# YanhaoWu/UMGen

Measured on AMD Instinct MI355X. Metric: scene_tokens_per_sec, higher is better.
Workload: dtype bf16; 1 GPU; UMGen_large --infer_task video, 5-frame rollout, 1 scene(s)/GPU, T=20 history frames, top-k 5/5/16 sampling, rule_constrain; scenes_per_gpu=1, history_frames=20, input_history_frames=20

## Files before the change

umgen_amd/csrc/debug_gemm_attn.hip:

```cpp
#include "debug_util.h"

namespace {
GemmArgs linear_args(const void* dW, const void* dA, int R, int N, int K, void* dO) {
    GemmArgs g{};
    g.P = dW; g.Q = dA; g.Mi = N; g.Nj = R; g.K = K; g.ldp = K; g.ldq = K; g.batch = 1; g.out = dO; g.ldo = N;
    return g;
}
GemmArgs vt_args(const void* dA, const void* dW, int F, int S, int S_pad, int N, int K, void* dO) {
    GemmArgs g{};
    g.P = dA; g.Q = dW; g.Mi = S; g.Nj = N; g.K = K; g.ldp = K; g.ldq = K; g.strideP = (long)S * K; g.strideQ = 0; g.batch = F;
    g.mode = GEMM_VT; g.out = dO; g.ldo = S_pad; g.H = N / kHeadDim;
    return g;
}
inline int pad64(int S) { return ((S + 63) / 64) * 64; }
void lcg_operands(Scratch& s, size_t na, size_t nw, DevPtr& dA, DevPtr& dW) {
    std::vector<bf16_t> h;
    unsigned x = 12345u;
    fill_lcg(h, na, x, 1.0f);
    dA = s.in(h.data(), na * 2);
    fill_lcg(h, nw, x, 0.05f);
    dW = s.in(h.data(), nw * 2);
}
}

extern "C" {

int umgen_dbg_linear(int flags, const void* act, const void* W, const float* bias, int R, int N, int K, int gelu, int resid, void* out) {
    const int bf16 = flags & 3;
    const size_t es = bf16 ? 2 : 4, osz = (size_t)R * N * (resid ? 4 : es);
    Scratch s;
    const void *dA = s.in(act, (size_t)R * K * es), *dW = s.in(W, (size_t)N * K * es);
    const float* dB = s.in(bias, (size_t)N * 4);
    void* dO = resid ? s.in(out, osz) : s.raw((size_t)R * N * 4);
    if (s.rc) return s.rc;
    GemmArgs g = linear_args(dW, dA, R, N, K, dO);
    g.mode = resid ? GEMM_RESID : GEMM_STORE; g.bias = dB; g.gelu = gelu;
    g.tile256 = (flags & 16) ? 1 : ((flags & 32) ? -1 : 0);
    if (bf16) by_prec16(bf16, [&](auto t) { launch_gemm_mfma<decltype(t)>(nullptr, g); });
    else launch_gemm_valu<float, float>(nullptr, g);
    if (int rc = finish()) return rc;
    return down(out, dO, osz);
}

int umgen_dbg_linear_vt(int flags, const void* act, const void* W, const float* bias, int F, int S, int N, int K, void* out) {
    const int prec = flags & 3;
    if (prec != 1 && prec != 2) return UMGEN_E_UNSUPPORTED;
    const int S_pad = pad64(S);
    const size_t R = (size_t)F * S, osz = (size_t)F * N * S_pad * 2;
    Scratch s;
    const void *dA = s.in(act, R * K * 2), *dW = s.in(W, (size_t)N * K * 2);
    const float* dB = s.in(bias, (size_t)N * 4);
    void* dO = s.raw(osz);
    if (s.rc) return s.rc;
    (void)hipMemset(dO, 0, osz);
    GemmArgs g = vt_args(dA, dW, F, S, S_pad, N, K, dO);
    g.bias = dB;
    g.tile256 = (flags & 16) ? 1 : ((flags & 32) ? -1 : 0);
    by_prec16(prec, [&](auto t) { launch_gemm_mfma<decltype(t)>(nullptr, g); });
    if (int rc = finish()) return rc;
    return down(out, dO, osz);
}

int umgen_dbg_attn_spatial(int flags, const void* qk, const void* v, int F, int S, int H, void* y) {
    const int bf16 = flags & 3;
    if ((flags & 64) && (flags & 32)) return UMGEN_E_UNSUPPORTED;
    const int E = H * kHeadDim, S_pad = pad64(S);
    const size_t es = bf16 ? 2 : 4, R = (size_t)F * S;
    std::vector<unsigned char> vt((size_t)F * E * S_pad * es, 0);
    const unsigned char* vs = (const unsigned char*)v;
    for (int f = 0; f < F; ++f)
        for (int sr = 0; sr < S; ++sr)
            for (int c = 0; c < E; ++c)
                memcpy(&vt[(((size_t)f * E + c) * S_pad + sr) * es], &vs[(((size_t)f * S + sr) * E + c) * es], es);
    Scratch s;
    const void *dQK = s.in(qk, R * 2 * E * es), *dVT = s.in(vt.data(), vt.size());
    void* dY = s.out(R * E * es);
    if (s.rc) return s.rc;
    if (int rc = fill_nan(dY, R * E, bf16)) return rc;
    by_prec(bf16, [&](auto t) {
        typedef decltype(t) T;
        const T *q = (const T*)dQK, *vtp = (const T*)dVT;
        if constexpr (std::is_same<T, float>::value) {
            if (flags & 64) launch_attn_causal_f32(nullptr, q, vtp, (T*)dY, F, S, S_pad, H);
            else if (flags & 32) launch_attn_spatial_valu<float>(nullptr, q, vtp, (T*)dY, F, S, S_pad, H);
            else launch_attn_spatial_f32_mfma(nullptr, q, vtp, (T*)dY, F, S, S_pad, H);
        } else if (flags & 64) {
            launch_attn_causal_mfma<T>(nullptr, q, vtp, (T*)dY, F, S, S_pad, H);
        } else {
            launch_attn_spatial_mfma<T>(nullptr, q, vtp, (T*)dY, F, S, S_pad, H);
        }
    });
    if (int rc = s.finish()) return rc;
    return down(y, dY, R * E * es);
}

int umgen_dbg_attn_temporal(int bf16, const void* qkv, int B, int T, int S, int H, int split, void* y) {
    const int E = H * kHeadDim;
    const size_t es = bf16 ? 2 : 4, row = (size_t)3 * E * es, orow = (size_t)E * es;
    auto pass = [&](int t0, int Tn, TemporalRange tr) -> int {
        const size_t Rn = (size_t)B * Tn * S;
        std::vector<unsigned char> hq(Rn * row), hy(Rn * orow);
        for (int b = 0; b < B; ++b)
            memcpy(&hq[(size_t)b * Tn * S * row], (const unsigned char*)qkv + ((size_t)b * T + t0) * S * row, (size_t)Tn * S * row);
        Scratch s;
        const void* dQ = s.in(hq.data(), hq.size());
        void* dY = s.raw(hy.size());
        if (s.rc) return s.rc;
        by_prec(bf16, [&](auto t) { typedef decltype(t) TT; launch_attn_temporal<TT>(nullptr, (const TT*)dQ, (TT*)dY, B, Tn, S, H, tr); });
        if (int rc = finish()) return rc;
        if (down(hy.data(), dY, hy.size())) return UMGEN_E_HIP;
        for (int b = 0; b < B; ++b)
            memcpy((unsigned char*)y + ((size_t)b * T + t0) * S * orow, &hy[(size_t)b * Tn * S * orow], (size_t)Tn * S * orow);
        return UMGEN_OK;
    };
    if (split <= 0 || split >= T) return pass(0, T, TemporalRange{0, nullptr, 0, 0});
    const int Tcap = T + 1;
    Scratch s;
    void* dC = s.raw((size_t)B * Tcap * S * 2 * E * es);
    if (s.rc) return s.rc;
    if (int rc = pass(0, split, TemporalRange{0, dC, Tcap, 1})) return rc;
    return pass(split, T - split, TemporalRange{split, dC, Tcap, 0});
}

int umgen_dbg_attn_decode(int bf16, const float* q, const void* kv, int NQ, int L, int H, float* y) {
    const int E = H * kHeadDim;
    const size_t es = bf16 ? 2 : 4;
    std::vector<float> eye((size_t)E * E, 0.f);
    for (int i = 0; i < E; ++i) eye[(size_t)i * E + i] = 1.f;
    Scratch s;
    const float* dQ = s.in(q, (size_t)NQ * E * 4);
    const void *dKV = s.in(kv, (size_t)L * 2 * E * es), *dW = s.in(eye.data(), eye.size() * 4);
    float *dP = s.raw((size_t)NQ * H * kAttnRec * 4), *dX = s.raw((size_t)NQ * E * 4);
    if (s.rc) return s.rc;
    (void)hipMemset(dX, 0, (size_t)NQ * E * 4);
    by_prec(bf16, [&](auto t) {
        typedef decltype(t) T;
        launch_attn_partial<T>(nullptr, dQ, (const T*)dKV, 0, kHeadDim, 2L * E, E, NQ, NQ, H, nullptr, L, attn_nsplit(L), dP);
    });
    GemvResidArgs a{};
    a.part = dP; a.H = H; a.ns = attn_nsplit(L); a.W = dW; a.N = E; a.K = E; a.M = NQ; a.x = dX; a.ldx = E;
    launch_gemv_resid<float>(nullptr, a);
    if (int rc = finish()) return rc;
    return down(y, dX, (size_t)NQ * E * 4);
}

int umgen_dbg_gemm_bench(int R, int N, int K, int mode, int iters, float* ms) {
    Scratch s;
    DevPtr dA, dW;
    lcg_operands(s, (size_t)R * K, (size_t)N * K, dA, dW);
    void* dO = s.raw((size_t)R * N * 4);
    if (s.rc) return s.rc;
    (void)hipMemset(dO, 0, (size_t)R * N * 4);
    GemmArgs g = linear_args(dW, dA, R, N, K, dO);
    g.mode = mode & 15; g.gelu = (mode >> 4) & 1;
    g.tile256 = (mode & 64) ? -1 : ((mode & 32) ? 1 : 0);
    return time_launches(nullptr, 1, iters, 1, ms, [&](int) { launch_gemm_mfma<bf16_t>(nullptr, g); });
}

int umgen_dbg_gemm_vt_bench(int F, int S, int N, int K, int flag, int iters, float* ms) {
    const int S_pad = pad64(S);
    const size_t osz = (size_t)F * N * S_pad * 2;
    Scratch s;
    DevPtr dA, dW;
    lcg_operands(s, (size_t)F * S * K, (size_t)N * K, dA, dW);
    void* dO = s.raw(osz);
    if (s.rc) return s.rc;
    (void)hipMemset(dO, 0, osz);
    GemmArgs g = vt_args(dA, dW, F, S, S_pad, N, K, dO);
    g.tile256 = (flag & 64) ? -1 : ((flag & 32) ? 1 : 0);
    return time_launches(nullptr, 1, iters, 1, ms, [&](int) { launch_gemm_mfma<bf16_t>(nullptr, g); });
}

int umgen_dbg_gemm_stamps(unsigned long long* out16) { return gemm256_read_stamps(out16); }

int umgen_dbg_gemv(int bf16, const float* x, const float* ln_w, const void* W, const float* bias, int M, int N, int K, int gelu, float* out) {
    const size_t es = bf16 ? 2 : 4, osz = (size_t)M * N * 4;
    Scratch s;
    GemvArgs a{};
    a.x = s.in(x, (size_t)M * K * 4); a.ldx = K; a.ln_w = s.in(ln_w, (size_t)K * 4); a.W = s.in(W, (size_t)N * K * es); a.bias = s.in(bias, (size_t)N * 4);
    a.N = N; a.K = K; a.M = M; a.out_mode = gelu ? GEMV_OUT_GELU : GEMV_OUT_F32; a.out = s.raw(osz); a.ldo = N; a.E = K;
    if (s.rc) return s.rc;
    for (int rpb = 0; rpb <= (M > 1 ? 1 : 0); ++rpb) {
        std::vector<float> got((size_t)M * N);
        if (rpb) (void)hipMemset(a.out, 0, osz);
        a.rows_per_block = rpb;
        by_prec(bf16, [&](auto t) { launch_gemv<decltype(t)>(nullptr, a); });
        if (int rc = finish()) return rc;
        if (int rc = down(rpb ? got.data() : out, a.out, osz)) return rc;
        if (rpb && memcmp(got.data(), out, osz) != 0) return UMGEN_E_STATE;
    }
    return UMGEN_OK;
}

int umgen_dbg_sample_topk(const float* logits, int n, int V, int k, float temp, const float* u, int32_t* tokens, int32_t* overflow) {
    if (V > 8192 || V < 1 || n < 1) return UMGEN_E_INVALID;
    Scratch s;
    const float *dL = s.in(logits, (size_t)n * V * 4), *dU = s.in(u, (size_t)n * 4);
    int *dT = s.raw((size_t)n * 4), *dO = s.raw(4);
    if (s.rc) return s.rc;
    (void)hipMemset(dO, 0, 4);
    launch_sample_rows(nullptr, dL, V, k, temp, dU, dT, dO, n);
    if (int rc = finish()) return rc;
    if (int rc = down(tokens, dT, (size_t)n * 4)) return rc;
    return down(overflow, dO, 4);
}

int umgen_dbg_batched_layer_bench(int prec, int M, int L, int iters, float* us) {
    const int E = 768, H = 16, Lmax = 2304;
    if (prec != 1 && prec != 2) return UMGEN_E_INVALID;
    if (M < 1 || M > kRowsMaxM || L < 1 || L >= Lmax) return UMGEN_E_INVALID;
    const size_t wsz = (size_t)12 * E * E * 2, csz = (size_t)M * 2 * H * Lmax * kHeadDim * 2, xsz = (size_t)64 * E * 4;
    std::vector<unsigned short> hw(wsz / 2);
    for (size_t i = 0; i < hw.size(); ++i) hw[i] = (unsigned short)(0x3c00 + (i * 2654435761u >> 24)) & (prec == 1 ? 0x3cff : 0x2fff);
    std::vector<float> hx((size_t)64 * E, 0.25f), hl(E, 1.f), hb(4 * E, 0.f);
    for (size_t i = 0; i < hx.size(); ++i) hx[i] = 0.25f + 1e-3f * (float)(i % 97);
    Scratch s;
    const char* Wq = s.in(hw.data(), wsz);
    void* dC = s.raw(csz);
    float *dx = s.in(hx.data(), xsz), *dxr = s.in(hx.data(), xsz), *dq = s.raw(xsz), *da = s.raw(xsz), *dh = s.raw(4 * xsz);
    const float *dln = s.in(hl.data(), (size_t)E * 4), *db = s.in(hb.data(), (size_t)4 * E * 4);
    const int* dlen = s.in(&L, 4);
    if (s.rc) return s.rc;
    if (hipMemset(da, 0, xsz) != hipSuccess || hipMemset(dh, 0, 4 * xsz) != hipSuccess || hipMemset(dC, 0, csz) != hipSuccess) return UMGEN_E_HIP;
    Stream stream;
    if (!stream.s) return UMGEN_E_HIP;
    hipStream_t st = stream.s;
    const long cstride = (long)2 * H * Lmax * kHeadDim;
    auto run = [&](int which) {
        by_prec16(prec, [&](auto tag) {
            typedef decltype(tag) TT;
            RowsArgs r{};
            r.M = M; r.E = E;
            switch (which) {
                case 0: r.x = dx; r.ln_w = dln; r.W = Wq; r.bias = db; r.N = 3 * E; r.K = E; r.mode = ROWS_QKV; r.out = dq; r.ldo = E;
                        r.cache = dC; r.scene_stride = cstride; r.d_len = dlen; r.Lmax = Lmax; launch_rows_mfma<TT>(st, r); break;
                case 1: launch_attn_decode_batched<TT>(st, dq, (const TT*)dC, cstride, M, H, Lmax, dlen, da); break;
                case 2: r.x = da; r.W = Wq + (size_t)3 * E * E * 2; r.bias = db; r.N = E; r.K = E; r.mode = ROWS_RESID; r.out = dxr; r.ldo = E; r.out_frag = dx; launch_rows_mfma<TT>(st, r); break;
                case 3: r.x = dx; r.ln_w = dln; r.W = Wq + (size_t)4 * E * E * 2; r.N = 4 * E; r.K = E; r.mode = ROWS_GELU; r.out_frag = dh; launch_rows_mfma<TT>(st, r); break;
                default: r.x = dh; r.W = Wq + (size_t)8 * E * E * 2; r.N = E; r.K = 4 * E; r.mode = ROWS_RESID; r.out = dxr; r.ldo = E; r.out_frag = dx; launch_rows_mfma<TT>(st, r); break;
            }
        });
    };
    if (int rc = time_launches(st, 3, iters, 6, us, [&](int which) { if (which < 5) run(which); else for (int k = 0; k < 5; ++k) run(k); })) return rc;
    for (int i = 0; i < 6; ++i) us[i] *= 1000.f;
    return UMGEN_OK;
}

}
```

umgen_amd/csrc/gemm.hip:

```cpp
#include <cstdlib>

#include "bg_queue.h"
#include "kernels.h"

namespace umgen {

template <int MODE, typename TO>
__device__ inline void epilogue4(const GemmArgs& a, int z, int i0, int j, const float (&v)[4]) {
    if (j >= a.Nj || i0 >= a.Mi) return;
    if (MODE == GEMM_VT) {
        const float b = a.bias ? a.bias[j] : 0.f;
        TO* dst = reinterpret_cast<TO*>(a.out) + (((long)z * a.H + j / kHeadDim) * kHeadDim + j % kHeadDim) * a.ldo + i0;
        if (i0 + 3 < a.Mi) {
            float o[4] = {v[0] + b, v[1] + b, v[2] + b, v[3] + b};
            store4(dst, o);
        } else {
            for (int r = 0; r < 4 && i0 + r < a.Mi; ++r) dst[r] = Cvt<TO>::from_f(v[r] + b);
        }
        return;
    }
    float o[4];
#pragma unroll
    for (int r = 0; r < 4; ++r) {
        float t = v[r] + (a.bias ? a.bias[i0 + r] : 0.f);
// ... 43 lines not shown
        pp[it] = P + (long)gi * a.ldp + schunk * 8;
        qq[it] = Q + (long)gj * a.ldq + schunk * 8;
    }
    uint4 rp[4], rq[4];
    auto gload = [&](int k0) {
        const bool ok = (k0 + schunk * 8) < a.K;
#pragma unroll
        for (int it = 0; it < 4; ++it) {
            rp[it] = ok ? *reinterpret_cast<const uint4*>(pp[it] + k0) : make_uint4(0, 0, 0, 0);
            rq[it] = ok ? *reinterpret_cast<const uint4*>(qq[it] + k0) : make_uint4(0, 0, 0, 0);
        }
    };
    auto lstore = [&](int buf) {
        unsigned char* ldsP = lds[buf];
        unsigned char* ldsQ = lds[buf] + BM * BK * 2;
#pragma unroll
        for (int it = 0; it < 4; ++it) {
            int r = srow + 32 * it;
            *reinterpret_cast<uint4*>(ldsP + swz(r, schunk)) = rp[it];
            *reinterpret_cast<uint4*>(ldsQ + swz(r, schunk)) = rq[it];
        }
    };
    f32x4_t acc[4][4];
#pragma unroll
    for (int m = 0; m < 4; ++m)
#pragma unroll
        for (int n = 0; n < 4; ++n) acc[m][n] = f32x4_t{0.f, 0.f, 0.f, 0.f};

    const int frow = lane & 15, g = lane >> 4;
    const int nkt = (a.K + BK - 1) / BK;
    gload(0);
    lstore(0);
    if (nkt > 1) gload(BK);
    __syncthreads();
    for (int kt = 0; kt < nkt; ++kt) {
        const unsigned char* ldsP = lds[kt & 1];
        const unsigned char* ldsQ = lds[kt & 1] + BM * BK * 2;
#pragma unroll
        for (int kk = 0; kk < 2; ++kk) {
            vec8 af[4], bfr[4];
            const int c = kk * 4 + g;
#pragma unroll
            for (int m = 0; m < 4; ++m) af[m] = *reinterpret_cast<const vec8*>(ldsP + swz(wi * 64 + m * 16 + frow, c));
#pragma unroll
            for (int n = 0; n < 4; ++n) bfr[n] = *reinterpret_cast<const vec8*>(ldsQ + swz(wj * 64 + n * 16 + frow, c));
#pragma unroll
            for (int m = 0; m < 4; ++m)
#pragma unroll
                for (int n = 0; n < 4; ++n) acc[m][n] = Mma16<TT>::mfma(af[m], bfr[n], acc[m][n]);
        }
        if (kt + 1 < nkt) {
            lstore((kt + 1) & 1);
            if (kt + 2 < nkt) gload((kt + 2) * BK);
        }
        __syncthreads();
    }
#pragma unroll
    for (int m = 0; m < 4; ++m)
#pragma unroll
        for (int n = 0; n < 4; ++n) {
            const int i0 = i_base + wi * 64 + m * 16 + 4 * g;
            const int j = j_base + wj * 64 + n * 16 + frow;
            float v[4] = {acc[m][n][0], acc[m][n][1], acc[m][n][2], acc[m][n][3]};
            epilogue4<MODE, TT>(a, z, i0, j, v);
        }
}

template <typename TT>
__device__ __forceinline__ void store_tile_rows_bf16(const GemmArgs& a, int z, int ti, int tj, const f32x4_t (&acc)[4][2], unsigned char* stg,
                                                     int tid, int wi, int wj, int frow, int g) {
    asm volatile("" ::: "memory");
    __builtin_amdgcn_s_barrier();
#pragma unroll
    for (int m = 0; m < 4; ++m) {
        const int i0 = ti * BM + wi * 64 + m * 16 + 4 * g;
        float bb[4];
#pragma unroll
        for (int r = 0; r < 4; ++r) bb[r] = a.bias ? a.bias[i0 + r] : 0.f;
#pragma unroll
        for (int n = 0; n < 2; ++n) {
            float o[4];
#pragma unroll
            for (int r = 0; r < 4; ++r) {
                const float t = acc[m][n][r] + bb[r];
                o[r] = a.gelu ? gelu_fast(t) : t;
            }
            const int tl = wj * 32 + n * 16 + frow;
            const int pg = (wi * 16 + m * 4 + g) ^ frow;
            store4(reinterpret_cast<TT*>(stg + tl * 256 + pg * 8), o);
        }
    }
    asm volatile("s_waitcnt lgkmcnt(0)" ::: "memory");
    __builtin_amdgcn_s_barrier();
    TT* out = reinterpret_cast<TT*>(a.out) + (long)z * a.strideO + (long)ti * BM;
#pragma unroll
    for (int it = 0; it < 4; ++it) {
        const int idx = tid + 512 * it;
        const int tl = idx >> 4, q = idx & 15;
        const int pos = ((2 * q) ^ (tl & 15)) & ~1;
        uint4 v = *reinterpret_cast<const uint4*>(stg + tl * 256 + pos * 8);
        if (tl & 1) v = make_uint4(v.z, v.w, v.x, v.y);
        const int token = tj * BN + tl;
        if (token < a.Nj) {
            typedef unsigned int u32x4 __attribute__((ext_vector_type(4)));
            __builtin_nontemporal_store(u32x4{v.x, v.y, v.z, v.w}, reinterpret_cast<u32x4*>(out + (long)token * a.ldo + 8 * q));
        }
    }
    asm volatile("s_waitcnt lgkmcnt(0)" ::: "memory");
}

__device__ __forceinline__ void rmw_tile_rows_f32(const GemmArgs& a, int z, int ti, int tj, const f32x4_t (&acc)[4][2], unsigned char* stg,
                                                  int tid, int wi, int wj, int frow, int g) {
    float* xbase = reinterpret_cast<float*>(a.out) + (long)z * a.strideO + (long)ti * BM;
#pragma unroll
    for (int hf = 0; hf < 2; ++hf) {
        asm volatile("s_waitcnt lgkmcnt(0)" ::: "memory");
        __builtin_amdgcn_s_barrier();
        if ((wj >> 1) == hf) {
#pragma unroll
            for (int m = 0; m < 4; ++m) {
                const int i0 = ti * BM + wi * 64 + m * 16 + 4 * g;
                float bb[4];
#pragma unroll
                for (int r = 0; r < 4; ++r) bb[r] = a.bias ? a.bias[i0 + r] : 0.f;
#pragma unroll
                for (int n = 0; n < 2; ++n) {
                    const int tl = (wj & 1) * 32 + n * 16 + frow;
                    const int pg = (wi * 16 + m * 4 + g) ^ (tl & 7);
                    *reinterpret_cast<float4*>(stg + tl * 512 + pg * 16) =
                        make_float4(acc[m][n][0] + bb[0], acc[m][n][1] + bb[1], acc[m][n][2] + bb[2], acc[m][n][3] + bb[3]);
                }
            }
        }
        asm volatile("s_waitcnt lgkmcnt(0)" ::: "memory");
        __builtin_amdgcn_s_barrier();
#pragma unroll
        for (int it = 0; it < 4; ++it) {
            const int idx = tid + 512 * it;
            const int tl = idx >> 5, q = idx & 31;
            const float4 v = *reinterpret_cast<const float4*>(stg + tl * 512 + ((q ^ (tl & 7)) << 4));
            const int token = tj * BN + hf * 64 + tl;
            if (token < a.Nj) {
                float* x = xbase + (long)token * a.ldo + 4 * q;
                float c[4];
                load4(x, c);
                c[0] += v.x; c[1] += v.y; c[2] += v.z; c[3] += v.w;
                store4(x, c);
            }
        }
    }
    asm volatile("s_waitcnt lgkmcnt(0)" ::: "memory");
}

template <int MODE, typename TT>
__global__ __launch_bounds__(512) void gemm_bf16_glds_kernel(GemmArgs a, int nI, int nJ) {
    typedef typename Mma16<TT>::vec vec8;
    __shared__ __attribute__((aligned(16))) unsigned char lds[2][2 * BM * BK * 2];
    const int z = blockIdx.z;
    const int tid = threadIdx.x, lane = tid & 63, wave = tid >> 6;
    const int wi = wave >> 2, wj = wave & 3;
    const int b = blockIdx.x;
    const int xcd = b & 7, lb = b >> 3;
    const int hI = (nI + 1) >> 1, qJ = (nJ + 3) >> 2;
    const int ti = (xcd & 1) * hI + lb % hI, tj = (xcd >> 1) * qJ + lb / hI;
    if (ti >= nI || tj >= nJ || ti >= ((xcd & 1) + 1) * hI || tj >= ((xcd >> 1) + 1) * qJ) return;
    const int i_base = ti * BM, j_base = tj * BN;
    const TT* P = reinterpret_cast<const TT*>(a.P) + (long)z * a.strideP;
    const TT* Q = reinterpret_cast<const TT*>(a.Q) + (long)z * a.strideQ;
    const TT* pp[2];
    const TT* qq[2];
#pragma unroll
    for (int it = 0; it < 2; ++it) {
        const int r = (wave + 8 * it) * 8 + (lane >> 3);
        const int c = (lane & 7) ^ (r & 7);
        pp[it] = P + (long)min(i_base + r, a.Mi - 1) * a.ldp + c * 8;
        qq[it] = Q + (long)min(j_base + r, a.Nj - 1) * a.ldq + c * 8;
    }
    auto issue = [&](int buf, int k0) {
#pragma unroll
        for (int it = 0; it < 2; ++it) {
            unsigned char* dp = lds[buf] + (wave + 8 * it) * 1024;
            __builtin_amdgcn_global_load_lds((const void*)(pp[it] + k0), (__attribute__((address_space(3))) void*)dp, 16, 0, 0);
            __builtin_amdgcn_global_load_lds((const void*)(qq[it] + k0), (__attribute__((address_space(3))) void*)(dp + BM * BK * 2), 16, 0, 0);
        }
    };
    f32x4_t acc[4][2];
#pragma unroll
    for (int m = 0; m < 4; ++m)
#pragma unroll
        for (int n = 0; n < 2; ++n) acc[m][n] = f32x4_t{0.f, 0.f, 0.f, 0.f};
    const int frow = lane & 15, g = lane >> 4;
    const int nkt = a.K / BK;
    issue(0, 0);
    __syncthreads();
    for (int kt = 0; kt < nkt; ++kt) {
        if (kt + 1 < nkt) issue((kt + 1) & 1, (kt + 1) * BK);
        const unsigned char* ldsP = lds[kt & 1];
        const unsigned char* ldsQ = lds[kt & 1] + BM * BK * 2;
#pragma unroll
        for (int kk = 0; kk < 2; ++kk) {
            vec8 af[4], bfr[2];
            const int c = kk * 4 + g;
#pragma unroll
            for (int m = 0; m < 4; ++m) af[m] = *reinterpret_cast<const vec8*>(ldsP + swz(wi * 64 + m * 16 + frow, c));
#pragma unroll
            for (int n = 0; n < 2; ++n) bfr[n] = *reinterpret_cast<const vec8*>(ldsQ + swz(wj * 32 + n * 16 + frow, c));
#pragma unroll
            for (int m = 0; m < 4; ++m)
#pragma unroll
                for (int n = 0; n < 2; ++n) acc[m][n] = Mma16<TT>::mfma(af[m], bfr[n], acc[m][n]);
        }
        __syncthreads();
    }
    if (MODE == GEMM_STORE && a.Mi % BM == 0) {
        store_tile_rows_bf16<TT>(a, z, ti, tj, acc, lds[0], tid, wi, wj, frow, g);
        return;
    }
    if (MODE == GEMM_RESID && a.Mi % BM == 0) {
        rmw_tile_rows_f32(a, z, ti, tj, acc, lds[0], tid, wi, wj, frow, g);
        return;
    }
#pragma unroll
    for (int m = 0; m < 4; ++m)
#pragma unroll
        for (int n = 0; n < 2; ++n) {
            const int i0 = i_base + wi * 64 + m * 16 + 4 * g;
            const int j = j_base + wj * 32 + n * 16 + frow;
            float v[4] = {acc[m][n][0], acc[m][n][1], acc[m][n][2], acc[m][n][3]};
            epilogue4<MODE, TT>(a, z, i0, j, v);
        }
}

template <int MODE, typename TT>
__global__ __launch_bounds__(512) void gemm_bf16_pers_kernel(GemmArgs a, int nI, int nJ) {
    typedef typename Mma16<TT>::vec vec8;
    __shared__ __attribute__((aligned(16))) unsigned char lds[2][2 * BM * BK * 2];
    const int z = blockIdx.z;
    const int tid = threadIdx.x, lane = tid & 63, wave = tid >> 6;
    const int wi = wave >> 2, wj = wave & 3;
    const int hI = (nI + 1) >> 1, qJ = (nJ + 3) >> 2;
    const int total = 8 * hI * qJ;
    const TT* P = reinterpret_cast<const TT*>(a.P) + (long)z * a.strideP;
    const TT* Q = reinterpret_cast<const TT*>(a.Q) + (long)z * a.strideQ;
    auto decode = [&](int b, int& ti, int& tj) {
        const int xcd = b & 7, lb = b >> 3;
        ti = (xcd & 1) * hI + lb % hI;
        tj = (xcd >> 1) * qJ + lb / hI;
        return !(ti >= nI || tj >= nJ || ti >= ((xcd & 1) + 1) * hI || tj >= ((xcd >> 1) + 1) * qJ);
    };
    auto next_valid = [&](int b) {
        int ti, tj;
        while (b < total && !decode(b, ti, tj)) b += gridDim.x;
        return b;
    };
    struct Src { const TT* pp[2]; const TT* qq[2]; };
    auto sources = [&](int b) {
        int ti, tj;
        decode(b, ti, tj);
        Src s;
#pragma unroll
        for (int it = 0; it < 2; ++it) {
            const int r = (wave + 8 * it) * 8 + (lane >> 3);
            const int c = (lane & 7) ^ (r & 7);
            s.pp[it] = P + (long)min(ti * BM + r, a.Mi - 1) * a.ldp + c * 8;
            s.qq[it] = Q + (long)min(tj * BN + r, a.Nj - 1) * a.ldq + c * 8;
        }
        return s;
    };
    auto issue = [&](int buf, const Src& s, int k0) {
#pragma unroll
        for (int it = 0; it < 2; ++it) {
            unsigned char* dp = lds[buf] + (wave + 8 * it) * 1024;
            __builtin_amdgcn_global_load_lds((const void*)(s.pp[it] + k0), (__attribute__((address_space(3))) void*)dp, 16, 0, 0);
            __builtin_amdgcn_global_load_lds((const void*)(s.qq[it] + k0), (__attribute__((address_space(3))) void*)(dp + BM * BK * 2), 16, 0, 0);
        }
    };
    const int frow = lane & 15, g = lane >> 4;
    const int nkt = a.K / BK;
    int tile = next_valid(blockIdx.x);
    if (tile >= total) return;
    Src cur = sources(tile);
    int gs = 0;
    issue(0, cur, 0);
    while (tile < total) {
        const int nxt = next_valid(tile + gridDim.x);
        const bool has_next = nxt < total;
        Src nx = cur;
        if (has_next) nx = sources(nxt);
        f32x4_t acc[4][2];
#pragma unroll
        for (int m = 0; m < 4; ++m)
#pragma unroll
            for (int n = 0; n < 2; ++n) acc[m][n] = f32x4_t{0.f, 0.f, 0.f, 0.f};
        __syncthreads();
        for (int kt = 0; kt < nkt; ++kt) {
            if (kt + 1 < nkt) issue((gs + 1) & 1, cur, (kt + 1) * BK);
            else if (has_next) issue((gs + 1) & 1, nx, 0);
            const unsigned char* ldsP = lds[gs & 1];
            const unsigned char* ldsQ = lds[gs & 1] + BM * BK * 2;
#pragma unroll
            for (int kk = 0; kk < 2; ++kk) {
                vec8 af[4], bfr[2];
                const int c = kk * 4 + g;
#pragma unroll
                for (int m = 0; m < 4; ++m) af[m] = *reinterpret_cast<const vec8*>(ldsP + swz(wi * 64 + m * 16 + frow, c));
#pragma unroll
                for (int n = 0; n < 2; ++n) bfr[n] = *reinterpret_cast<const vec8*>(ldsQ + swz(wj * 32 + n * 16 + frow, c));
#pragma unroll
                for (int m = 0; m < 4; ++m)
#pragma unroll
                    for (int n = 0; n < 2; ++n) acc[m][n] = Mma16<TT>::mfma(af[m], bfr[n], acc[m][n]);
            }
            ++gs;
            if (kt + 1 < nkt) __syncthreads();
        }
        int ti, tj;
        decode(tile, ti, tj);
        if (MODE == GEMM_STORE && a.Mi % BM == 0) {
            store_tile_rows_bf16<TT>(a, z, ti, tj, acc, lds[(gs - 1) & 1], tid, wi, wj, frow, g);
        } else if (MODE == GEMM_RESID && a.Mi % BM == 0) {
            rmw_tile_rows_f32(a, z, ti, tj, acc, lds[(gs - 1) & 1], tid, wi, wj, frow, g);
        } else {
#pragma unroll
            for (int m = 0; m < 4; ++m)
#pragma unroll
                for (int n = 0; n < 2; ++n) {
                    const int i0 = ti * BM + wi * 64 + m * 16 + 4 * g;
                    const int j = tj * BN + wj * 32 + n * 16 + frow;
                    float v[4] = {acc[m][n][0], acc[m][n][1], acc[m][n][2], acc[m][n][3]};
                    epilogue4<MODE, TT>(a, z, i0, j, v);
                }
        }
        tile = nxt;
        cur = nx;
    }
}

template <typename TT>
void launch_gemm_mfma(hipStream_t s, const GemmArgs& a) {
    if (g_bg_rec) {
        GemmArgs v = a;
        if (a.mode == GEMM_VT) {
            v.P = a.Q; v.Mi = a.Nj; v.ldp = a.ldq; v.strideP = a.strideQ;
            v.Q = a.P; v.Nj = a.Mi; v.ldq = a.ldp; v.strideQ = a.strideP;
        }
        record_gemm256(v);
        return;
    }
    static const int min_tiles256 = getenv("UMGEN_GEMM256_MIN_TILES") ? atoi(getenv("UMGEN_GEMM256_MIN_TILES")) : 300;
    const long tiles256 = (long)(a.Mi / 256) * ((a.Nj + 255) / 256);
    if (a.tile256 >= 0 && gemm256_supported(a) && (a.tile256 > 0 || tiles256 >= min_tiles256 || (a.K >= 2048 && tiles256 >= min_tiles256 / 3))) {
        launch_gemm256<TT>(s, a);
        return;
    }
    if (a.mode == GEMM_VT && a.tile256 >= 0) {
        GemmArgs v = a;
        v.P = a.Q; v.Mi = a.Nj; v.ldp = a.ldq; v.strideP = a.strideQ;
        v.Q = a.P; v.Nj = a.Mi; v.ldq = a.ldp; v.strideQ = a.strideP;
        const long tiles = (long)(v.Mi / 256) * ((v.Nj + 255) / 256) * v.batch;
        if (gemm256_supported(v) && (a.tile256 > 0 || tiles >= min_tiles256)) {
            launch_gemm256<TT>(s, v);
            return;
        }
    }
    const int nI = (a.Mi + BM - 1) / BM, nJ = (a.Nj + BN - 1) / BN;
    dim3 grid(((nJ + 7) / 8) * 8 * nI, 1, a.batch), block(256);
    if (a.K % BK == 0 && a.batch == 1 && a.mode != GEMM_VT && (long)nI * nJ >= 1024) {
        static int n_cu = 0;
        if (!n_cu) {
            int dev = 0;
            hipDeviceProp_t prop;
            n_cu = (hipGetDevice(&dev) == hipSuccess && hipGetDeviceProperties(&prop, dev) == hipSuccess) ? prop.multiProcessorCount : 256;
        }
        const dim3 pg(2 * n_cu, 1, 1), block8(512);
        switch (a.mode) {
            case GEMM_STORE: hipLaunchKernelGGL((gemm_bf16_pers_kernel<GEMM_STORE, TT>), pg, block8, 0, s, a, nI, nJ); break;
            case GEMM_RESID: hipLaunchKernelGGL((gemm_bf16_pers_kernel<GEMM_RESID, TT>), pg, block8, 0, s, a, nI, nJ); break;
            default: hipLaunchKernelGGL((gemm_bf16_pers_kernel<GEMM_STORE_F32, TT>), pg, block8, 0, s, a, nI, nJ); break;
        }
        return;
    }
    if (a.K % BK == 0) {
        grid = dim3(8 * ((nI + 1) / 2) * ((nJ + 3) / 4), 1, a.batch);
        const dim3 block8(512);
        switch (a.mode) {
            case GEMM_STORE: hipLaunchKernelGGL((gemm_bf16_glds_kernel<GEMM_STORE, TT>), grid, block8, 0, s, a, nI, nJ); break;
            case GEMM_RESID: hipLaunchKernelGGL((gemm_bf16_glds_kernel<GEMM_RESID, TT>), grid, block8, 0, s, a, nI, nJ); break;
            case GEMM_STORE_F32: hipLaunchKernelGGL((gemm_bf16_glds_kernel<GEMM_STORE_F32, TT>), grid, block8, 0, s, a, nI, nJ); break;
            default: hipLaunchKernelGGL((gemm_bf16_glds_kernel<GEMM_VT, TT>), grid, block8, 0, s, a, nI, nJ); break;
        }
        return;
    }
    switch (a.mode) {
        case GEMM_STORE: hipLaunchKernelGGL((gemm_bf16_mfma_kernel<GEMM_STORE, TT>), grid, block, 0, s, a, nI, nJ); break;
        case GEMM_RESID: hipLaunchKernelGGL((gemm_bf16_mfma_kernel<GEMM_RESID, TT>), grid, block, 0, s, a, nI, nJ); break;
        case GEMM_STORE_F32: hipLaunchKernelGGL((gemm_bf16_mfma_kernel<GEMM_STORE_F32, TT>), grid, block, 0, s, a, nI, nJ); break;
        default: hipLaunchKernelGGL((gemm_bf16_mfma_kernel<GEMM_VT, TT>), grid, block, 0, s, a, nI, nJ); break;
    }
}
template void launch_gemm_mfma<bf16_t>(hipStream_t, const GemmArgs&);
template void launch_gemm_mfma<f16_t>(hipStream_t, const GemmArgs&);

template <int MODE, typename TP, typename TQ, typename TO>
__global__ __launch_bounds__(256) void gemm_valu_kernel(GemmArgs a) {
    __shared__ float sP[16][64 + 4];
    __shared__ float sQ[16][64 + 4];
    const int z = blockIdx.z;
    const int tid = threadIdx.x;
    const int i_base = blockIdx.x * 64, j_base = blockIdx.y * 64;
    const TP* P = reinterpret_cast<const TP*>(a.P) + (long)z * a.strideP;
    const TQ* Q = reinterpret_cast<const TQ*>(a.Q) + (long)z * a.strideQ;
    const int ti = tid & 15, tj = tid >> 4;
    float acc[4][4] = {};
    const int lr = tid >> 2, lk = (tid & 3) * 4;
    for (int k0 = 0; k0 < a.K; k0 += 16) {
        {
            const int gi = min(i_base + lr, a.Mi - 1), gj = min(j_base + lr, a.Nj - 1);
#pragma unroll
            for (int e = 0; e < 4; ++e) {
                const int k = k0 + lk + e;
                sP[lk + e][lr] = (k < a.K) ? Cvt<TP>::to_f(P[(long)gi * a.ldp + k]) : 0.f;
                sQ[lk + e][lr] = (k < a.K) ? Cvt<TQ>::to_f(Q[(long)gj * a.ldq + k]) : 0.f;
            }
        }
        __syncthreads();
#pragma unroll
        for (int k = 0; k < 16; ++k) {
            float p[4], q[4];
#pragma unroll
            for (int r = 0; r < 4; ++r) p[r] = sP[k][4 * ti + r];
#pragma unroll
            for (int c = 0; c < 4; ++c) q[c] = sQ[k][4 * tj + c];
#pragma unroll
            for (int r = 0; r < 4; ++r)
#pragma unroll
                for (int c = 0; c < 4; ++c) acc[r][c] = fmaf(p[r], q[c], acc[r][c]);
        }
        __syncthreads();
    }
#pragma unroll
    for (int c = 0; c < 4; ++c) {
        float v[4] = {acc[0][c], acc[1][c], acc[2][c], acc[3][c]};
        epilogue4<MODE, TO>(a, z, i_base + 4 * ti, j_base + 4 * tj + c, v);
    }
}

constexpr int FM = 128, FK = 32, FLD = FM + 4;
template <int MODE, typename TO>
__global__ __launch_bounds__(256) void gemm_f32_mfma_kernel(GemmArgs a) {
    __shared__ __attribute__((aligned(16))) float sP[2][FK][FLD];
    __shared__ __attribute__((aligned(16))) float sQ[2][FK][FLD];
    const int z = blockIdx.z;
    const int tid = threadIdx.x, lane = tid & 63, wave = tid >> 6;
    const int wi = wave >> 1, wj = wave & 1;
    const int i_base = blockIdx.x * FM, j_base = blockIdx.y * FM;
    const float* P = reinterpret_cast<const float*>(a.P) + (long)z * a.strideP;
    const float* Q = reinterpret_cast<const float*>(a.Q) + (long)z * a.strideQ;
    const int lr = tid >> 3, lk = (tid & 7) * 4;
    const bool k4 = (a.K % 4 == 0) && (a.ldp % 4 == 0) && (a.ldq % 4 == 0) && (a.strideP % 4 == 0) && (a.strideQ % 4 == 0) &&
                    (((uintptr_t)a.P | (uintptr_t)a.Q) % 16 == 0);
    float4 rp[4], rq[4];
    auto fetch = [&](int k0) {
#pragma unroll
        for (int it = 0; it < 4; ++it) {
            const int gi = min(i_base + lr + 32 * it, a.Mi - 1), gj = min(j_base + lr + 32 * it, a.Nj - 1);
            const float* pp = P + (long)gi * a.ldp + k0 + lk;
            const float* qq = Q + (long)gj * a.ldq + k0 + lk;
            if (k4 && k0 + lk + 3 < a.K) {
                rp[it] = *reinterpret_cast<const float4*>(pp);
                rq[it] = *reinterpret_cast<const float4*>(qq);
            } else {
                float tp[4], tq[4];
#pragma unroll
                for (int e = 0; e < 4; ++e) {
                    const bool in = k0 + lk + e < a.K;
                    tp[e] = in ? pp[e] : 0.f;
                    tq[e] = in ? qq[e] : 0.f;
                }
                rp[it] = make_float4(tp[0], tp[1], tp[2], tp[3]);
                rq[it] = make_float4(tq[0], tq[1], tq[2], tq[3]);
            }
        }
    };
    auto stash = [&](int buf) {
#pragma unroll
        for (int it = 0; it < 4; ++it) {
            const int r = lr + 32 * it;
            sP[buf][lk + 0][r] = rp[it].x; sP[buf][lk + 1][r] = rp[it].y; sP[buf][lk + 2][r] = rp[it].z; sP[buf][lk + 3][r] = rp[it].w;
            sQ[buf][lk + 0][r] = rq[it].x; sQ[buf][lk + 1][r] = rq[it].y; sQ[buf][lk + 2][r] = rq[it].z; sQ[buf][lk + 3][r] = rq[it].w;
        }
    };
    f32x16_t acc[2][2];
#pragma unroll
    for (int m = 0; m < 2; ++m)
#pragma unroll
        for (int n = 0; n < 2; ++n)
#pragma unroll
            for (int r = 0; r < 16; ++r) acc[m][n][r] = 0.f;
    fetch(0);
    stash(0);
    __syncthreads();
    const int l32 = lane & 31, lk2 = lane >> 5;
    int buf = 0;
    for (int k0 = 0; k0 < a.K; k0 += FK) {
        const bool more = k0 + FK < a.K;
        if (more) fetch(k0 + FK);
        const int kmax = min(FK, a.K - k0);
        for (int kk = 0; kk < kmax; kk += 2) {
            const float a0 = sP[buf][kk + lk2][wi * 64 + l32], a1 = sP[buf][kk + lk2][wi * 64 + 32 + l32];
            const float b0 = sQ[buf][kk + lk2][wj * 64 + l32], b1 = sQ[buf][kk + lk2][wj * 64 + 32 + l32];
#if defined(__HIP_DEVICE_COMPILE__)
            acc[0][0] = __builtin_amdgcn_mfma_f32_32x32x2f32(a0, b0, acc[0][0], 0, 0, 0);
            acc[0][1] = __builtin_amdgcn_mfma_f32_32x32x2f32(a0, b1, acc[0][1], 0, 0, 0);
            acc[1][0] = __builtin_amdgcn_mfma_f32_32x32x2f32(a1, b0, acc[1][0], 0, 0, 0);
            acc[1][1] = __builtin_amdgcn_mfma_f32_32x32x2f32(a1, b1, acc[1][1], 0, 0, 0);
#endif
        }
        if (more) {
            stash(buf ^ 1);
            __syncthreads();
            buf ^= 1;
        }
    }
#pragma unroll
    for (int m = 0; m < 2; ++m)
#pragma unroll
        for (int n = 0; n < 2; ++n)
#pragma unroll
            for (int q = 0; q < 4; ++q) {
                const int i0 = i_base + wi * 64 + m * 32 + 8 * q + 4 * lk2;
                const int j = j_base + wj * 64 + n * 32 + l32;
                float v[4] = {acc[m][n][4 * q], acc[m][n][4 * q + 1], acc[m][n][4 * q + 2], acc[m][n][4 * q + 3]};
                epilogue4<MODE, TO>(a, z, i0, j, v);
            }
}

static bool use_f32_mfma() {
    static const bool on = !(getenv("UMGEN_FP32_MFMA") && getenv("UMGEN_FP32_MFMA")[0] == '0');
    return on;
}

template <>
void launch_gemm_valu<float, float>(hipStream_t s, const GemmArgs& a) {
    if (use_f32_mfma() && a.tile256 >= 0 && a.Mi % 4 == 0) {
        dim3 grid((a.Mi + FM - 1) / FM, (a.Nj + FM - 1) / FM, a.batch), block(256);
        switch (a.mode) {
            case GEMM_STORE: hipLaunchKernelGGL((gemm_f32_mfma_kernel<GEMM_STORE, float>), grid, block, 0, s, a); break;
            case GEMM_RESID: hipLaunchKernelGGL((gemm_f32_mfma_kernel<GEMM_RESID, float>), grid, block, 0, s, a); break;
            case GEMM_STORE_F32: hipLaunchKernelGGL((gemm_f32_mfma_kernel<GEMM_STORE_F32, float>), grid, block, 0, s, a); break;
            default: hipLaunchKernelGGL((gemm_f32_mfma_kernel<GEMM_VT, float>), grid, block, 0, s, a); break;
        }
        return;
    }
    dim3 grid((a.Mi + 63) / 64, (a.Nj + 63) / 64, a.batch), block(256);
// ... 25 lines not shown
```

umgen_amd/csrc/kernels.h:

```cpp
#pragma once
#include "common.h"

namespace umgen {

enum GemmMode {
    GEMM_STORE = 0,
    GEMM_RESID = 1,
    GEMM_STORE_F32 = 2,
    GEMM_VT = 3
};
struct GemmArgs {
    const void* P; const void* Q;
    int Mi, Nj, K;
    long ldp, ldq;
    long strideP, strideQ;
    int batch;
    int mode;
    const float* bias;
    int gelu;
    void* out;
    long ldo;
    long strideO;
    int H;
    int tile256;
};
bool gemm256_supported(const GemmArgs& a);
hipError_t gemm256_prepare();
int gemm256_read_stamps(unsigned long long* out16);
template <typename TT> void launch_gemm256(hipStream_t s, const GemmArgs& a);
void record_gemm256(const GemmArgs& a);
template <typename TT> void launch_gemm_mfma(hipStream_t s, const GemmArgs& a);
template <typename TP, typename TQ> void launch_gemm_valu(hipStream_t s, const GemmArgs& a);

template <typename T> void launch_layernorm(hipStream_t s, const float* x, long row_stride, long n_rows, int E, const float* w, T* out);

template <typename TT> void launch_attn_spatial_mfma(hipStream_t s, const TT* qk, const TT* vt, TT* y, int F, int S, int S_pad, int H);
template <typename T> void launch_attn_spatial_valu(hipStream_t s, const T* qk, const T* vt, T* y, int F, int S, int S_pad, int H);
void launch_attn_spatial_f32_mfma(hipStream_t s, const float* qk, const float* vt, float* y, int F, int S, int S_pad, int H);
template <typename TT> void launch_attn_causal_mfma(hipStream_t s, const TT* qk, const TT* vt, TT* y, int F, int S, int S_pad, int H);
void launch_attn_causal_f32(hipStream_t s, const float* qk, const float* vt, float* y, int F, int S, int S_pad, int H);
struct TemporalRange { int t0; void* cache; int Tcap; int write; int q0 = 0; };
template <typename T> void launch_attn_temporal(hipStream_t s, const T* qkv, T* y, int B, int Tn, int S, int H,
                                                TemporalRange tr = TemporalRange{0, nullptr, 0, 0});

constexpr int kAttnSplit = 18;
constexpr int kAttnChunk = 128;
inline int attn_nsplit(int L) { return L <= 0 ? 1 : (L + kAttnChunk - 1) / kAttnChunk; }
constexpr int kAttnPad = 20;
constexpr int kAttnRec = 2 * kAttnPad + kHeadDim * kAttnPad;
template <typename T> void launch_attn_partial(hipStream_t s, const float* q, const T* kv_base, long scene_stride, long head_stride,
                                               long key_stride, long v_off, int NQ, int q_per_scene, int H, const int* d_len, int len_add,
                                               int ns, float* part);

enum GemvOut {
    GEMV_OUT_F32 = 0,
    GEMV_OUT_GELU = 1,
    GEMV_OUT_QKV = 2
};
struct GemvArgs {
    const float* x; long ldx;
    const int* d_xoff; long xoff_mul;
    const float* ln_w;
    const void* W; const float* bias; int N, K, M;
    int out_mode;
    float* out; long ldo;
    void* cache; long scene_stride; const int* d_len; int Lmax;
    int rows_per_block;
    int E;
};
template <typename T> void launch_gemv(hipStream_t s, const GemvArgs& a);

struct GemvResidArgs {
    const float* a; long lda; const float* part; int H;
    int ns;
    const void* W; const float* bias; int N, K, M;
    float* x; long ldx;
    int rows_per_block;
};
template <typename T> void launch_gemv_resid(hipStream_t s, const GemvResidArgs& a);

struct DecodeLayerArgs {
    const float *ln_a, *bqkv, *bo, *ln_b;
    const void *Wqkv, *Wo, *Wfc, *Wproj;
    float* x;
    float *q, *h, *part;
    void* cache; long scene_stride; int Lmax; const int* d_len;
    int B, E, H, ns, rows_per_block;
};
template <typename T> void launch_decode_layer(hipStream_t s, const DecodeLayerArgs& a);

inline int ego_cross_nsplit() { return attn_nsplit(kSeq); }
inline void launch_ego_self_attn(hipStream_t s, const float* q, const float* qkv3, int M, int H, float* part) {
    const int E = H * kHeadDim;
    launch_attn_partial<float>(s, q, qkv3 + E, 3L * 3 * E, kHeadDim, 3L * E, E, M, 3, H, nullptr, 3, 1, part);
}
template <typename T>
void launch_ego_cross_attn(hipStream_t s, const float* q, const T* kv, int M, int H, float* part) {
    const int E = H * kHeadDim;
    launch_attn_partial<T>(s, q, kv, (long)kSeq * 2 * E, kHeadDim, 2L * E, E, M, 3, H, nullptr, kSeq, ego_cross_nsplit(), part);
}

enum RowsMode {
    ROWS_F32 = 0,
    ROWS_GELU = 1,
    ROWS_QKV = 2,
    ROWS_RESID = 3
};
constexpr int kRowsMaxM = 64;
constexpr int kRowsMaxNB = 4;
__host__ __device__ inline long frag_index(int m, int k) {
    return ((((long)(k >> 5) * kRowsMaxNB + (m >> 4)) * 64 + ((k & 31) >> 3) * 16 + (m & 15)) << 3) + (k & 7);
}
struct RowsArgs {
    const float* x; int M;
    const float* ln_w;
    const void* W; const float* bias; int N, K;
    int mode;
    float* out; long ldo;
    float* out_frag;
    void* cache; long scene_stride; const int* d_len; int Lmax; int E;
};
template <typename TT> void launch_rows_mfma(hipStream_t s, const RowsArgs& a);
void launch_rows_to_frag(hipStream_t s, const float* x, long ldx, int M, int K, float* xf);
template <typename TT> void launch_attn_decode_batched(hipStream_t s, const float* q, const TT* cache, long scene_stride, int B, int H, int Lmax,
                                                        const int* d_len, float* y);

struct HeadNllArgs {
    const float* x; long ldx; int rows_per_group; long group_stride;
    const float* ln_w;
    const void* W; int V, K, M;
    const int* target; long target_group_stride;
    float* part;
    float* logp; int* argmax;
    float *lse, *tlogit;
};
inline bool head_nll_supported(int K) { return K == 96 || K == 768 || K == 1536; }
__host__ __device__ inline int head_nll_tiles_per_split(int V) { const int nt = (V + 15) / 16, t = (nt + 7) / 8; return t < 13 ? 13 : t; }
inline int head_nll_nsplit(int V) { const int nt = (V + 15) / 16, t = head_nll_tiles_per_split(V); return (nt + t - 1) / t; }
template <typename T> hipError_t launch_head_nll(hipStream_t s, const HeadNllArgs& a);
void launch_logits_nll(hipStream_t s, const float* logits, long ld, int V, int M, const int* target, int rows_per_group, long target_group_stride,
                       float* logp, int* argmax, float* lse, float* tlogit);

constexpr int kEngE = 768, kEngH = 16;
constexpr int kEngThreads = 512;
constexpr int kEngGroup = 32;
constexpr int kEngWpUnits = 18;
constexpr int kEngLocStride = 3 * kEngE + 2 * kEngH * 50 + kEngE + kEngGroup * kEngE + kEngE;
struct OarLayerDev {
    const bf16_t *Wqkv, *Wo, *Wfc, *Wproj;
    const bf16_t *Wp2;
    const float *bqkv, *bo, *ln_a, *ln_b;
    const bf16_t *Wf2;
};
struct OarState;
struct BgQueue;
struct OarEngineArgs {
    const OarLayerDev* layers; int n_layers;
    bf16_t* kvcache; long kv_layer_stride, kv_scene_stride; int Lmax;
    long unused_[3];
    float* xdec;
    const OarState* st;
    unsigned long long* gx;
    unsigned long long* gloc;
    unsigned int* ticket;
    unsigned int* err;
    int B, NG, R, D;
    unsigned char xcc_group[16];
    unsigned long long* stamps;
    int fp16;
    int systolic;
    int burn_ticks, burn_mfma, burn_sleep, burn_kb;
    const void* burn_buf;
    BgQueue* bg;
    int bg_only;
};
constexpr int kWideE = 1536;
constexpr int kWideGroups = 256;
constexpr int kWideSplits = 4;
struct OarWideArgs {
    const OarLayerDev* layers; int n_layers;
    bf16_t* kvcache; long kv_layer_stride, kv_scene_stride; int Lmax;
    float* xdec;
    int scene;
    const OarState* st;
// ... 20 lines not shown
```

Measured before the change: 2003 scene-tokens/s.

## Add three-stage LDS ring pipeline to global-load-LDS GEMM for small grids

Generalizes the glds GEMM kernel from a fixed double buffer to an NS-slot ring buffer in dynamic shared memory. Prefetching two tiles ahead uses partial vmcnt waits so global loads overlap more MFMA work. The three-stage path is chosen automatically when the grid fits in one wave of CUs (blocks <= CU count), with debug flags to force a depth. The cost is more LDS per block, which can reduce occupancy, plus per-device attribute setup on the host.

```diff
diff --git a/umgen_amd/csrc/debug_gemm_attn.hip b/umgen_amd/csrc/debug_gemm_attn.hip
--- a/umgen_amd/csrc/debug_gemm_attn.hip
+++ b/umgen_amd/csrc/debug_gemm_attn.hip
@@ -13,6 +13,7 @@
     return g;
 }
 inline int pad64(int S) { return ((S + 63) / 64) * 64; }
+inline int ring_of(int flags) { return (flags & 128) ? 2 : ((flags & 256) ? 3 : 0); }
 void lcg_operands(Scratch& s, size_t na, size_t nw, DevPtr& dA, DevPtr& dW) {
     std::vector<bf16_t> h;
     unsigned x = 12345u;
@@ -36,7 +37,7 @@
     GemmArgs g = linear_args(dW, dA, R, N, K, dO);
     g.mode = resid ? GEMM_RESID : GEMM_STORE; g.bias = dB; g.gelu = gelu;
     g.tile256 = (flags & 16) ? 1 : ((flags & 32) ? -1 : 0);
-    if (bf16) by_prec16(bf16, [&](auto t) { launch_gemm_mfma<decltype(t)>(nullptr, g); });
+    if (bf16) by_prec16(bf16, [&](auto t) { launch_gemm_mfma<decltype(t)>(nullptr, g, ring_of(flags)); });
     else launch_gemm_valu<float, float>(nullptr, g);
     if (int rc = finish()) return rc;
     return down(out, dO, osz);
@@ -56,7 +57,7 @@
     GemmArgs g = vt_args(dA, dW, F, S, S_pad, N, K, dO);
     g.bias = dB;
     g.tile256 = (flags & 16) ? 1 : ((flags & 32) ? -1 : 0);
-    by_prec16(prec, [&](auto t) { launch_gemm_mfma<decltype(t)>(nullptr, g); });
+    by_prec16(prec, [&](auto t) { launch_gemm_mfma<decltype(t)>(nullptr, g, ring_of(flags)); });
     if (int rc = finish()) return rc;
     return down(out, dO, osz);
 }
@@ -154,7 +155,8 @@
     GemmArgs g = linear_args(dW, dA, R, N, K, dO);
     g.mode = mode & 15; g.gelu = (mode >> 4) & 1;
     g.tile256 = (mode & 64) ? -1 : ((mode & 32) ? 1 : 0);
-    return time_launches(nullptr, 1, iters, 1, ms, [&](int) { launch_gemm_mfma<bf16_t>(nullptr, g); });
+    const int ring = ring_of(mode);
+    return time_launches(nullptr, 1, iters, 1, ms, [&](int) { launch_gemm_mfma<bf16_t>(nullptr, g, ring); });
 }
 
 int umgen_dbg_gemm_vt_bench(int F, int S, int N, int K, int flag, int iters, float* ms) {
@@ -168,7 +170,8 @@
     (void)hipMemset(dO, 0, osz);
     GemmArgs g = vt_args(dA, dW, F, S, S_pad, N, K, dO);
     g.tile256 = (flag & 64) ? -1 : ((flag & 32) ? 1 : 0);
-    return time_launches(nullptr, 1, iters, 1, ms, [&](int) { launch_gemm_mfma<bf16_t>(nullptr, g); });
+    const int ring = ring_of(flag);
+    return time_launches(nullptr, 1, iters, 1, ms, [&](int) { launch_gemm_mfma<bf16_t>(nullptr, g, ring); });
 }
 
 int umgen_dbg_gemm_stamps(unsigned long long* out16) { return gemm256_read_stamps(out16); }
diff --git a/umgen_amd/csrc/gemm.hip b/umgen_amd/csrc/gemm.hip
--- a/umgen_amd/csrc/gemm.hip
+++ b/umgen_amd/csrc/gemm.hip
@@ -219,10 +219,29 @@
     asm volatile("s_waitcnt lgkmcnt(0)" ::: "memory");
 }
 
-template <int MODE, typename TT>
+constexpr int kRingSlot = 2 * BM * BK * 2;
+
+template <int N>
+__device__ __forceinline__ void ring_wait(int n) {
+    if constexpr (N == 0) {
+        asm volatile("s_waitcnt vmcnt(0)" ::: "memory");
+    } else {
+        if (n >= N) asm volatile("s_waitcnt vmcnt(%0)" ::"n"(4 * N) : "memory");
+        else ring_wait<N - 1>(n);
+    }
+}
+
+template <int MODE, typename TT, int NS>
 __global__ __launch_bounds__(512) void gemm_bf16_glds_kernel(GemmArgs a, int nI, int nJ) {
     typedef typename Mma16<TT>::vec vec8;
-    __shared__ __attribute__((aligned(16))) unsigned char lds[2][2 * BM * BK * 2];
+    unsigned char* lds;
+    if constexpr (NS == 2) {
+        __shared__ __attribute__((aligned(16))) unsigned char lds2[2 * kRingSlot];
+        lds = lds2;
+    } else {
+        extern __shared__ __attribute__((aligned(1024))) unsigned char lds_ring[];
+        lds = lds_ring;
+    }
     const int z = blockIdx.z;
     const int tid = threadIdx.x, lane = tid & 63, wave = tid >> 6;
     const int wi = wave >> 2, wj = wave & 3;
@@ -243,10 +262,10 @@
         pp[it] = P + (long)min(i_base + r, a.Mi - 1) * a.ldp + c * 8;
         qq[it] = Q + (long)min(j_base + r, a.Nj - 1) * a.ldq + c * 8;
     }
-    auto issue = [&](int buf, int k0) {
+    auto issue = [&](int slot, int k0) {
 #pragma unroll
         for (int it = 0; it < 2; ++it) {
-            unsigned char* dp = lds[buf] + (wave + 8 * it) * 1024;
+            unsigned char* dp = lds + slot * kRingSlot + (wave + 8 * it) * 1024;
             __builtin_amdgcn_global_load_lds((const void*)(pp[it] + k0), (__attribute__((address_space(3))) void*)dp, 16, 0, 0);
             __builtin_amdgcn_global_load_lds((const void*)(qq[it] + k0), (__attribute__((address_space(3))) void*)(dp + BM * BK * 2), 16, 0, 0);
         }
@@ -258,12 +277,9 @@
         for (int n = 0; n < 2; ++n) acc[m][n] = f32x4_t{0.f, 0.f, 0.f, 0.f};
     const int frow = lane & 15, g = lane >> 4;
     const int nkt = a.K / BK;
-    issue(0, 0);
-    __syncthreads();
-    for (int kt = 0; kt < nkt; ++kt) {
-        if (kt + 1 < nkt) issue((kt + 1) & 1, (kt + 1) * BK);
-        const unsigned char* ldsP = lds[kt & 1];
-        const unsigned char* ldsQ = lds[kt & 1] + BM * BK * 2;
+    auto multiply = [&](int slot) {
+        const unsigned char* ldsP = lds + slot * kRingSlot;
+        const unsigned char* ldsQ = ldsP + BM * BK * 2;
 #pragma unroll
         for (int kk = 0; kk < 2; ++kk) {
             vec8 af[4], bfr[2];
@@ -277,14 +293,38 @@
 #pragma unroll
                 for (int n = 0; n < 2; ++n) acc[m][n] = Mma16<TT>::mfma(af[m], bfr[n], acc[m][n]);
         }
+    };
+    if constexpr (NS == 2) {
+        issue(0, 0);
         __syncthreads();
+        for (int kt = 0; kt < nkt; ++kt) {
+            if (kt + 1 < nkt) issue((kt + 1) & 1, (kt + 1) * BK);
+            multiply(kt & 1);
+            __syncthreads();
+        }
+    } else {
+#pragma unroll
+        for (int t = 0; t < NS - 1; ++t)
+            if (t < nkt) issue(t, t * BK);
+        int rs = 0, ws = NS - 1;
+        for (int kt = 0; kt < nkt; ++kt) {
+            ring_wait<NS - 2>(nkt - 1 - kt);
+            asm volatile("s_waitcnt lgkmcnt(0)" ::: "memory");
+            __builtin_amdgcn_s_barrier();
+            if (kt + NS - 1 < nkt) issue(ws, (kt + NS - 1) * BK);
+            multiply(rs);
+            rs = rs + 1 == NS ? 0 : rs + 1;
+            ws = ws + 1 == NS ? 0 : ws + 1;
+        }
+        asm volatile("s_waitcnt lgkmcnt(0)" ::: "memory");
+        __builtin_amdgcn_s_barrier();
     }
     if (MODE == GEMM_STORE && a.Mi % BM == 0) {
-        store_tile_rows_bf16<TT>(a, z, ti, tj, acc, lds[0], tid, wi, wj, frow, g);
+        store_tile_rows_bf16<TT>(a, z, ti, tj, acc, lds, tid, wi, wj, frow, g);
         return;
     }
     if (MODE == GEMM_RESID && a.Mi % BM == 0) {
-        rmw_tile_rows_f32(a, z, ti, tj, acc, lds[0], tid, wi, wj, frow, g);
+        rmw_tile_rows_f32(a, z, ti, tj, acc, lds, tid, wi, wj, frow, g);
         return;
     }
 #pragma unroll
@@ -403,8 +443,44 @@
     }
 }
 
+template <typename TT, int NS>
+void launch_glds(hipStream_t s, const GemmArgs& a, dim3 grid, int nI, int nJ) {
+    const dim3 block8(512);
+    const size_t dyn = NS > 2 ? (size_t)NS * kRingSlot : 0;
+    if (NS > 2) {
+        static bool ready[64] = {};
+        int dev = 0;
+        if (hipGetDevice(&dev) != hipSuccess || dev < 0 || dev >= 64) dev = 0;
+        if (!ready[dev]) {
+            const void* fns[] = {reinterpret_cast<const void*>(gemm_bf16_glds_kernel<GEMM_STORE, TT, NS>), reinterpret_cast<const void*>(gemm_bf16_glds_kernel<GEMM_RESID, TT, NS>),
+                                 reinterpret_cast<const void*>(gemm_bf16_glds_kernel<GEMM_STORE_F32, TT, NS>), reinterpret_cast<const void*>(gemm_bf16_glds_kernel<GEMM_VT, TT, NS>)};
+            bool ok = true;
+            for (const void* f : fns) ok = hipFuncSetAttribute(f, hipFuncAttributeMaxDynamicSharedMemorySize, (int)dyn) == hipSuccess && ok;
+            ready[dev] = ok;
+        }
+    }
+    switch (a.mode) {
+        case GEMM_STORE: hipLaunchKernelGGL((gemm_bf16_glds_kernel<GEMM_STORE, TT, NS>), grid, block8, dyn, s, a, nI, nJ); break;
+        case GEMM_RESID: hipLaunchKernelGGL((gemm_bf16_glds_kernel<GEMM_RESID, TT, NS>), grid, block8, dyn, s, a, nI, nJ); break;
+        case GEMM_STORE_F32: hipLaunchKernelGGL((gemm_bf16_glds_kernel<GEMM_STORE_F32, TT, NS>), grid, block8, dyn, s, a, nI, nJ); break;
+        default: hipLaunchKernelGGL((gemm_bf16_glds_kernel<GEMM_VT, TT, NS>), grid, block8, dyn, s, a, nI, nJ); break;
+    }
+}
+
+static int cu_count() {
+    static int n_cu = 0;
+    if (!n_cu) {
+        int dev = 0;
+        hipDeviceProp_t prop;
+        n_cu = (hipGetDevice(&dev) == hipSuccess && hipGetDeviceProperties(&prop, dev) == hipSuccess) ? prop.multiProcessorCount : 256;
+    }
+    return n_cu;
+}
+
+static int ring_depth(long blocks) { return blocks <= cu_count() ? 3 : 2; }
+
 template <typename TT>
-void launch_gemm_mfma(hipStream_t s, const GemmArgs& a) {
+void launch_gemm_mfma(hipStream_t s, const GemmArgs& a, int ring) {
     if (g_bg_rec) {
         GemmArgs v = a;
         if (a.mode == GEMM_VT) {
@@ -433,13 +509,7 @@
     const int nI = (a.Mi + BM - 1) / BM, nJ = (a.Nj + BN - 1) / BN;
     dim3 grid(((nJ + 7) / 8) * 8 * nI, 1, a.batch), block(256);
     if (a.K % BK == 0 && a.batch == 1 && a.mode != GEMM_VT && (long)nI * nJ >= 1024) {
-        static int n_cu = 0;
-        if (!n_cu) {
-            int dev = 0;
-            hipDeviceProp_t prop;
-            n_cu = (hipGetDevice(&dev) == hipSuccess && hipGetDeviceProperties(&prop, dev) == hipSuccess) ? prop.multiProcessorCount : 256;
-        }
-        const dim3 pg(2 * n_cu, 1, 1), block8(512);
+        const dim3 pg(2 * cu_count(), 1, 1), block8(512);
         switch (a.mode) {
             case GEMM_STORE: hipLaunchKernelGGL((gemm_bf16_pers_kernel<GEMM_STORE, TT>), pg, block8, 0, s, a, nI, nJ); break;
             case GEMM_RESID: hipLaunchKernelGGL((gemm_bf16_pers_kernel<GEMM_RESID, TT>), pg, block8, 0, s, a, nI, nJ); break;
@@ -449,13 +519,8 @@
     }
     if (a.K % BK == 0) {
         grid = dim3(8 * ((nI + 1) / 2) * ((nJ + 3) / 4), 1, a.batch);
-        const dim3 block8(512);
-        switch (a.mode) {
-            case GEMM_STORE: hipLaunchKernelGGL((gemm_bf16_glds_kernel<GEMM_STORE, TT>), grid, block8, 0, s, a, nI, nJ); break;
-            case GEMM_RESID: hipLaunchKernelGGL((gemm_bf16_glds_kernel<GEMM_RESID, TT>), grid, block8, 0, s, a, nI, nJ); break;
-            case GEMM_STORE_F32: hipLaunchKernelGGL((gemm_bf16_glds_kernel<GEMM_STORE_F32, TT>), grid, block8, 0, s, a, nI, nJ); break;
-            default: hipLaunchKernelGGL((gemm_bf16_glds_kernel<GEMM_VT, TT>), grid, block8, 0, s, a, nI, nJ); break;
-        }
+        if ((ring ? ring : ring_depth((long)grid.x * a.batch)) == 3) launch_glds<TT, 3>(s, a, grid, nI, nJ);
+        else launch_glds<TT, 2>(s, a, grid, nI, nJ);
         return;
     }
     switch (a.mode) {
@@ -465,8 +530,8 @@
         default: hipLaunchKernelGGL((gemm_bf16_mfma_kernel<GEMM_VT, TT>), grid, block, 0, s, a, nI, nJ); break;
     }
 }
-template void launch_gemm_mfma<bf16_t>(hipStream_t, const GemmArgs&);
-template void launch_gemm_mfma<f16_t>(hipStream_t, const GemmArgs&);
+template void launch_gemm_mfma<bf16_t>(hipStream_t, const GemmArgs&, int);
+template void launch_gemm_mfma<f16_t>(hipStream_t, const GemmArgs&, int);
 
 template <int MODE, typename TP, typename TQ, typename TO>
 __global__ __launch_bounds__(256) void gemm_valu_kernel(GemmArgs a) {
diff --git a/umgen_amd/csrc/kernels.h b/umgen_amd/csrc/kernels.h
--- a/umgen_amd/csrc/kernels.h
+++ b/umgen_amd/csrc/kernels.h
@@ -29,7 +29,7 @@
 int gemm256_read_stamps(unsigned long long* out16);
 template <typename TT> void launch_gemm256(hipStream_t s, const GemmArgs& a);
 void record_gemm256(const GemmArgs& a);
-template <typename TT> void launch_gemm_mfma(hipStream_t s, const GemmArgs& a);
+template <typename TT> void launch_gemm_mfma(hipStream_t s, const GemmArgs& a, int ring = 0);
 template <typename TP, typename TQ> void launch_gemm_valu(hipStream_t s, const GemmArgs& a);
 
 template <typename T> void launch_layernorm(hipStream_t s, const float* x, long row_stride, long n_rows, int E, const float* w, T* out);
```

After: 1971 scene-tokens/s. 0.984x the previous value.
